# librosa/librosa

Measured on NVIDIA H100. Metric: mel-spectrogram frames/sec (n_fft=2048,hop=512,n_mels=128), higher is better.
Workload: dtype f32

## Files before the change

librosa_b200/csrc/api.cu:

```cuda
#include <cuda_runtime.h>
#include <math.h>
#include <stdlib.h>
#include <string.h>

#include <algorithm>

#include "aux_kernels.cuh"
#include "czt_kernel.cuh"
#include "feat_kernels.cuh"
#include "internal.h"
#include "mr_kernel.cuh"
#include "pitch_kernels.cuh"

using namespace b2l;

#define B2L_CASE(L) case L: return fwd_kernel_##L(variant, mode);
static FwdKernel fwd_kernel_for(int log2m, int variant, int mode) {
  switch (log2m) { B2L_FFT_SIZES(B2L_CASE) }
  return nullptr;
}
#undef B2L_CASE
#define B2L_CASE(L) case L: return inv_kernel_##L(variant);
static InvKernel inv_kernel_for(int log2m, int variant) {
  switch (log2m) { B2L_FFT_SIZES(B2L_CASE) }
  return nullptr;
}
#undef B2L_CASE
#define B2L_CASE(L) case L: return czt_kernel_##L();
static CztKernel czt_kernel_for(int log2p) {
  switch (log2p) { B2L_CZT_SIZES(B2L_CASE) }
  return nullptr;
}
#undef B2L_CASE
#define B2L_CASE(L) case L: return czt_inv_kernel_##L();
static CztInvKernel czt_inv_kernel_for(int log2p) {
  switch (log2p) { B2L_CZT_SIZES(B2L_CASE) }
  return nullptr;
}
#undef B2L_CASE

static int cta_variants(const HostFftCfg& cfg, int out[3]) {
  int n = 0;
  if (cfg.log2m >= 9 && cfg.log2m <= 11) out[n++] = 116;
  int nws[2];
  const int k = cfg.nw_options(nws);
  for (int i = 0; i < k; ++i) out[n++] = nws[i];
  return n;
}
static int variant_threads(int variant) { return variant == 116 ? 512 : variant * 32; }

enum Path { PATH_POW2, PATH_MR, PATH_CZT, PATH_NONE };
enum Entry {
  ENTRY_SPECTRUM,
  ENTRY_MEL,
  ENTRY_STATS,
};
static bool mr_enabled(const b2l_plan* p) {
  if (p->log2p == 0) return true;
  const char* e = getenv("B2L_MR");
  return !(e && *e) || atoi(e) != 0;
}
static Path route(const b2l_plan* p, Entry entry) {
  if (!p->czt) return PATH_POW2;
  switch (entry) {
    case ENTRY_SPECTRUM: return p->mr && mr_enabled(p) ? PATH_MR : PATH_CZT;
    case ENTRY_MEL: return p->mr ? PATH_MR : PATH_NONE;
    default: return PATH_NONE;
  }
}

static int frame_count(b2l_ctx* c, const b2l_plan* p, int64_t n_clips, int64_t n, int64_t y_stride, const float* d_y,
                       const void* d_out, long long* T) {
  if (p->ctx != c) return fail(B2L_ERR_INVALID, "plan belongs to another context");
  if (n_clips < 0 || n < 0 || y_stride < n) return fail(B2L_ERR_INVALID, "bad clip geometry");
  if (n > 0x7fffffffLL) return fail(B2L_ERR_UNSUPPORTED, "clips longer than 2^31-1 samples are not supported");
  *T = plan_frames(p, n);
  if (*T <= 0)
    return fail(B2L_ERR_INVALID, "n_fft=%d is too large for input signal of length=%lld", p->n_fft, (long long)n);
  if (n_clips == 0) *T = 0;
  else if (!d_y || !d_out) return fail(B2L_ERR_INVALID, "NULL device pointer");
  return B2L_OK;
}

struct StatsCall { StatsParams sp; const float* d_freq; };

static int run_forward(b2l_ctx* c, const b2l_plan* p, int mode, int log_mode, const float* d_y, int64_t n_clips,
                       int64_t n, int64_t y_stride, float2* out_c, float* out_r, const StatsCall* stats = nullptr) {
  long long T = 0;
  int rc = frame_count(c, p, n_clips, n, y_stride, d_y, mode == MODE_STFT ? (void*)out_c : (void*)out_r, &T);
  if (rc || T == 0) return rc;
  if (mode == MODE_MEL && p->n_mels == 0) return fail(B2L_ERR_INVALID, "plan has no mel stage");
  DeviceGuard g(c->device);

  HostFftCfg cfg(p->log2m);
  const int N = p->n_fft, M = N / 2;
  int variants[3];
  const int n_opt = cta_variants(cfg, variants);
  FwdArgs a;
  memset(&a, 0, sizeof(a));
  int variant = 0, ft = 0, halves = 1;
  size_t smem = 0;
  const b2l_plan::RowTable* rt = nullptr;
  for (int i = 0; i < n_opt && !variant; ++i) {
    const int v = variants[i];
    const int nh = v == 116 ? 2 : 1;
    const int nw = nh > 1 ? 16 : v;
    if (nw * 32 % (cfg.tpf * nh) != 0) continue;
    const int f = nw * 32 / nh / cfg.tpf;
    if (f < 1 || f > 32) continue;
    const long long span = (long long)(f - 1) * p->hop + N;
    if (span > 0x3fffffff) continue;
    const b2l_plan::RowTable* t = nullptr;
    if (mode == MODE_MEL) {
      rc = get_row_table(p, mel_rows_per_warp(f), &t);
      if (rc) return rc;
    }
    size_t off = 0;
    a.off_win = (int)off; off = align_up(off + (size_t)N * 4, 16);
    a.off_tw = (int)off; off = align_up(off + (size_t)cfg.tw_count(true) * 8, 16);
    a.off_bar = (int)off; off = align_up(off + 8 * nh, 16);
    if (t) {
      a.off_melw = (int)off; off = align_up(off + (size_t)t->w_count * 4, 16);
      a.off_melband = (int)off; off = align_up(off + (size_t)t->n_rows * sizeof(MelRow), 16);
    }
    if (mode == MODE_STATS) {
      a.off_melw = (int)off; off = align_up(off + (size_t)(M + 1) * 4, 16);
    }
    a.off_in = (int)(off = align_up(off, 128));
    a.in_stride = (int)align_up((size_t)span * 4, 128);
    off += (size_t)a.in_stride * nh;
    a.off_xbuf = (int)(off = align_up(off, 128));
    size_t xbytes = (size_t)f * cfg.xbuf_f2() * 8;
    if (mode == MODE_MEL || mode == MODE_STATS) {
      xbytes = (size_t)f * mel_group_stride(M, f) * 8 + (M < 128 ? (size_t)(M + 16) * 4 : 0);
    }
    a.xbuf_stride = (int)align_up(xbytes, 128);
    off += (size_t)a.xbuf_stride * nh;
    if (off > c->smem_optin) continue;
    variant = v;
    ft = f;
    halves = nh;
    smem = off;
    rt = t;
    a.in_floats = (int)span;
  }
  if (!variant)
    return fail(B2L_ERR_UNSUPPORTED, "hop_length=%d with n_fft=%d needs more shared memory than one SM has", p->hop,
                p->n_fft);

  a.y = d_y;
  a.clip_stride = y_stride;
  a.n = (int)n;
  a.n_clips = (int)n_clips;
  a.n_fft = N;
  a.hop = p->hop;
  a.pad = p->center ? N / 2 : 0;
  a.pad_mode = p->pad_mode;
  a.n_frames = (int)T;
  a.tiles_per_clip = (int)((T + ft - 1) / ft);
  a.total_tiles = (long long)a.tiles_per_clip * n_clips;
  a.tma_ok = (((uintptr_t)d_y & 15) == 0) && (y_stride % 4 == 0) && (a.in_floats % 4 == 0);
  a.window = p->d_win_fwd;
  a.tw = p->d_tw_fwd;
  a.twn = p->d_twn;
  a.out_c = out_c;
  a.out_r = out_r;
  a.power_mode = p->power_mode;
  a.power = p->power;
  a.n_mels = p->n_mels;
  if (mode == MODE_STATS) {
    if (!stats || !stats->d_freq) return fail(B2L_ERR_INVALID, "NULL frequency table");
    a.power_mode = 1;
    a.power = 1.0f;
    a.stats = stats->sp;
    a.mel_w = stats->d_freq;
    a.mel_w_count = M + 1;
  }
  if (rt) {
    a.mel_w_count = rt->w_count;
    a.mel_w = rt->d_w;
    a.mel_rows = rt->d_rows;
    a.n_mel_rows = rt->n_rows;
  }
  a.log_mode = log_mode ? 1 : 0;
  a.out_tiled = log_mode == 2 ? 1 : 0;
  a.amin = p->amin;
  a.db_sub = 10.0f * log10f(fmaxf(p->amin, fabsf(p->ref_value)));
  a.clip_max = c->d_clip_max;
  a.status = c->d_status;

  const FwdKernel fn = fwd_kernel_for(p->log2m, variant, mode);
  if (!fn) return fail(B2L_ERR_CUDA, "no forward kernel variant %d for n_fft=%d", variant, N);
  const int threads = variant_threads(variant);
  int occ = 0;
  if ((rc = blocks_per_sm(c, fn, threads, smem, &occ))) return rc;
  if (occ < 1) return fail(B2L_ERR_CUDA, "forward kernel does not fit on an SM (smem %zu)", smem);
  long long grid = (long long)c->sm_count * occ;
  const long long ctas_needed = (a.total_tiles + halves - 1) / halves;
  if (grid > ctas_needed) grid = ctas_needed;
  return launch(c, fn, (unsigned)grid, threads, smem, a);
}

static size_t czt_smem(const b2l_plan* p, const HostFftCfg& cfg, int G, bool forward) {
  const size_t bins = forward ? (size_t)(1 + p->n_fft / 2) : 0;
  return (size_t)((cfg.tw_count() + 15) & ~15) * 8 + (size_t)G * cfg.xbuf_f2() * 8 +
         ((size_t)(1 << p->log2p) + (size_t)((p->n_fft + 1) & ~1) + bins) * 8;
}

static int run_czt(b2l_ctx* c, const b2l_plan* p, int mode, const float* d_y, int64_t n_clips, int64_t n,
                   int64_t y_stride, float2* out_c, float* out_r) {
  long long T = 0;
  int rc = frame_count(c, p, n_clips, n, y_stride, d_y, mode == 0 ? (void*)out_c : (void*)out_r, &T);
  if (rc || T == 0) return rc;
  DeviceGuard g(c->device);
  HostFftCfg cfg(p->log2p);
  const int nw = cfg.czt_nw();
  const int G = nw * 32 / cfg.tpf;
  CztArgs a;
  memset(&a, 0, sizeof(a));
  a.y = d_y;
  a.clip_stride = y_stride;
  a.n = (int)n;
  a.n_clips = (int)n_clips;
  a.L = p->n_fft;
  a.hop = p->hop;
  a.pad = p->center ? p->n_fft / 2 : 0;
  a.pad_mode = p->pad_mode;
  a.n_frames = (int)T;
  a.n_bins = 1 + p->n_fft / 2;
  a.wb = p->d_czt_wb;
  a.bk = p->d_czt_bk;
  a.hf = p->d_czt_hf;
  a.out_c = out_c;
  a.out_r = out_r;
  a.mode = mode;
  a.power_mode = p->power_mode;
  a.power = p->power;
  a.status = c->d_status;
  const size_t smem = czt_smem(p, cfg, G, true);
  const CztKernel fn = czt_kernel_for(p->log2p);
  int occ = 0;
  if ((rc = blocks_per_sm(c, fn, nw * 32, c->smem_optin / 2 + 1, &occ))) return rc;
  if (smem > c->smem_optin) return fail(B2L_ERR_UNSUPPORTED, "n_fft=%d needs more shared memory than one SM has", p->n_fft);
  if (occ < 1) return fail(B2L_ERR_CUDA, "chirp-z kernel does not fit on an SM (smem %zu)", smem);
  const long long steps = ((long long)n_clips * ((T + 1) / 2) + G - 1) / G;
  long long grid = (long long)c->sm_count * occ;
  if (grid > steps) grid = steps;
  return launch(c, fn, (unsigned)grid, nw * 32, smem, a);
}

static int mr_block(const b2l_ctx* c, const b2l_plan* p, int n_mels, int mel_w_count, int fpw, int* nw, size_t* smem) {
  const size_t tables = mr_table_bytes(p->n_fft, p->mr_tw_count, n_mels, mel_w_count);
  const size_t per_warp = (size_t)2 * (p->n_fft / 2) * sizeof(float2) * (size_t)fpw;
  const size_t budget = (c->smem_optin + 1024) / 2 - 1024;
  int w = 16;
  while (w > 1 && tables + w * per_warp > budget) --w;
  if (tables + w * per_warp > c->smem_optin)
    return fail(B2L_ERR_UNSUPPORTED, "n_fft=%d needs more shared memory than one SM has", p->n_fft);
  *nw = w;
  *smem = tables + w * per_warp;
  return B2L_OK;
}

static int run_mr(b2l_ctx* c, const b2l_plan* p, int mode, int log_mode, const float* d_y, int64_t n_clips, int64_t n,
                  int64_t y_stride, float2* out_c, float* out_r) {
  long long T = 0;
  int rc = frame_count(c, p, n_clips, n, y_stride, d_y, mode == 0 ? (void*)out_c : (void*)out_r, &T);
  if (rc || T == 0) return rc;
  if (mode == 2 && p->n_mels == 0) return fail(B2L_ERR_INVALID, "plan has no mel stage");
  if (n_clips > 0x7fffffffLL || T > 0x7fffffffLL) return fail(B2L_ERR_UNSUPPORTED, "batch too large");
  DeviceGuard g(c->device);
  MrArgs a;
  memset(&a, 0, sizeof(a));
  a.y = d_y;
  a.clip_stride = y_stride;
  a.n = (int)n;
// ... 1032 lines not shown
```

librosa_b200/csrc/common.cuh:

```cuda
#pragma once
#include <cuda_runtime.h>
#include <stdint.h>

namespace b2l {

enum PadMode : int {
  PAD_CONSTANT = 0,
  PAD_EDGE = 1,
  PAD_REFLECT = 2,
  PAD_SYMMETRIC = 3,
  PAD_LINEAR_RAMP = 4,
  PAD_EMPTY = 5,
};

enum FwdMode : int {
  MODE_STFT = 0,
  MODE_MEL = 1,
  MODE_SPEC = 2,
  MODE_STATS = 3,
};

constexpr int kMrMaxPass = 12;

struct MelBand { int lo, len, off, pad; };
struct MelRow { unsigned short lo, quads; unsigned int off; };

template <int M, int FT>
struct MelLayout {
  static constexpr bool PAIR = (FT % 2) == 0 && FT >= 8;
  static constexpr int FP = PAIR ? FT / 2 : FT;
  static constexpr int H = 32 / FP;
  static constexpr int RSM = H < 4 ? 4 : H;
  static constexpr int XB = M + M / 32;
  static constexpr int GS = XB + ((((RSM - 2 * XB) % 32) + 32) % 32) / 2;
  static constexpr int RS = 2 * GS;
  static_assert(RS >= M + 4 && RS % 32 == RSM % 32 && RS % 4 == 0, "row stride");
};
__host__ __device__ inline int mel_rows_per_warp(int ft) { return 32 / (((ft % 2) == 0 && ft >= 8) ? ft / 2 : ft); }
__host__ __device__ inline int mel_group_stride(int m, int ft) {
  const int h = mel_rows_per_warp(ft), rsm = h < 4 ? 4 : h, xb = m + m / 32;
  return xb + ((((rsm - 2 * xb) % 32) + 32) % 32) / 2;
}

enum StatRow : int { STAT_CENTROID = 0, STAT_BANDWIDTH = 1, STAT_ROLLOFF = 2, STAT_FLATNESS = 3, STAT_RMS = 4, STAT_TOTAL = 5 };
constexpr int N_STATS = 6;
struct StatsParams {
  float roll_percent;
  float flat_amin, flat_power;
  float bw_p;
  int bw_norm;
  int frame_length;
  int want;
};

struct FwdArgs {
  const float* y;
  long long clip_stride;
  int n, n_clips;
  int n_fft, hop, pad, pad_mode, n_frames;
  int tiles_per_clip;
  long long total_tiles;
  int tma_ok;
  const float* window;
  const float2* tw;
  const float2* twn;
  float2* out_c;
  float* out_r;
  int power_mode;
  float power;
  int n_mels, mel_w_count;
  const float* mel_w;
  const MelRow* mel_rows;
  int n_mel_rows;
  int log_mode;
  int out_tiled;
  float amin, db_sub;
  unsigned int* clip_max;
  int* status;
  StatsParams stats;
  int off_win, off_tw, off_in, off_xbuf, off_melw, off_melband, off_bar;
  int in_stride, xbuf_stride;
  int in_floats;
};

struct InvArgs {
  const float2* D;
  long long d_clip_stride;
  int n_clips, n_frames;
  int n_fft, hop, start;
  int out_len;
  long long y_clip_stride;
  float* y;
  const float* window;
  const float* inv_wss;
  const float2* tw;
  const float2* twn;
  int frames_per_slot;
  int vec4;
  int off_win, off_tw, off_xbuf, off_acc;
  int xbuf_stride, acc_stride;
  int acc_floats;
};

__host__ __device__ inline unsigned int float_to_key(float f) {
#ifdef __CUDA_ARCH__
  unsigned int u = __float_as_uint(f);
#else
  union { float f; unsigned int u; } c; c.f = f; unsigned int u = c.u;
#endif
  return (u & 0x80000000u) ? ~u : (u | 0x80000000u);
}
__host__ __device__ inline float key_to_float(unsigned int k) {
  unsigned int u = (k & 0x80000000u) ? (k & 0x7fffffffu) : ~k;
#ifdef __CUDA_ARCH__
  return __uint_as_float(u);
#else
  union { float f; unsigned int u; } c; c.u = u; return c.f;
#endif
}

}
```

librosa_b200/csrc/fwd_inst.cu:

```cuda
#include "fwd_kernel.cuh"
#include "internal.h"

#ifndef B2L_LOG2M
#error "compile with -DB2L_LOG2M=<2..12>"
#endif

namespace b2l {
namespace {

template <int L, int TPF, int NW, int DUAL>
FwdKernel by_mode(int mode) {
  switch (mode) {
    case MODE_STFT: return fwd_kernel<L, TPF, NW, MODE_STFT, DUAL>;
    case MODE_MEL: return fwd_kernel<L, TPF, NW, MODE_MEL, DUAL>;
    case MODE_SPEC: return fwd_kernel<L, TPF, NW, MODE_SPEC, DUAL>;
    case MODE_STATS: return fwd_kernel<L, TPF, NW, MODE_STATS, DUAL>;
  }
  return nullptr;
}

template <int L>
FwdKernel variant_kernel(int variant, int mode) {
  constexpr int M = 1 << L;
  constexpr int TPF = M >= 32 ? M / 32 : 1;
  if constexpr (L >= 10) {
    if (variant == 16) return by_mode<L, TPF, 16, 1>(mode);
    if (variant == 8) return by_mode<L, TPF, 8, 1>(mode);
    if (variant == 116) return by_mode<L, TPF, 16, 2>(mode);
  } else {
    constexpr int NW = TPF > 16 ? 16 : TPF;
    if (variant == NW) return by_mode<L, TPF, NW, 1>(mode);
    if constexpr (L == 9) {
      if (variant == 116) return by_mode<L, TPF, 16, 2>(mode);
    }
  }
  return nullptr;
}

}

#define B2L_CAT2(a, b) a##b
#define B2L_CAT(a, b) B2L_CAT2(a, b)

FwdKernel B2L_CAT(fwd_kernel_, B2L_LOG2M)(int variant, int mode) { return variant_kernel<B2L_LOG2M>(variant, mode); }

}
```

librosa_b200/csrc/fwd_kernel.cuh:

```cuda
#pragma once
#include "common.cuh"
#include "fft_engine.cuh"
#include "stats.cuh"


namespace b2l {

__device__ __forceinline__ void mbar_init(uint64_t* bar, int count) {
  asm volatile("mbarrier.init.shared::cta.b64 [%0], %1;" ::"r"(smem_u32(bar)), "r"(count) : "memory");
}
__device__ __forceinline__ void fence_mbar_init() {
  asm volatile("fence.mbarrier_init.release.cluster;" ::: "memory");
}
__device__ __forceinline__ void fence_proxy_async() {
  asm volatile("fence.proxy.async.shared::cta;" ::: "memory");
}
__device__ __forceinline__ void mbar_expect_tx(uint64_t* bar, uint32_t bytes) {
  asm volatile("mbarrier.arrive.expect_tx.shared::cta.b64 _, [%0], %1;" ::"r"(smem_u32(bar)), "r"(bytes)
               : "memory");
}
__device__ __forceinline__ void mbar_wait(uint64_t* bar, uint32_t phase) {
  asm volatile(
      "{\n\t"
      ".reg .pred p;\n\t"
      "WAIT_%=:\n\t"
      "mbarrier.try_wait.parity.shared::cta.b64 p, [%0], %1;\n\t"
      "@p bra DONE_%=;\n\t"
      "bra WAIT_%=;\n\t"
      "DONE_%=:\n\t"
      "}" ::"r"(smem_u32(bar)), "r"(phase)
      : "memory");
}
__device__ __forceinline__ void tma_load_1d(void* dst_smem, const void* src_gmem, uint32_t bytes, uint64_t* bar) {
  asm volatile(
      "cp.async.bulk.shared::cluster.global.mbarrier::complete_tx::bytes [%0], [%1], %2, [%3];" ::"r"(
          smem_u32(dst_smem)),
      "l"(src_gmem), "r"(bytes), "r"(smem_u32(bar))
      : "memory");
}

__device__ __forceinline__ float load_padded(const float* __restrict__ y, int n, long long j, int mode, int pad) {
  if (j >= 0 && j < n) return __ldg(y + j);
  switch (mode) {
    case PAD_EDGE:
      return __ldg(y + (j < 0 ? 0 : n - 1));
    case PAD_REFLECT: {
      if (n == 1) return __ldg(y);
      long long P = 2LL * (n - 1);
      long long m = j % P;
      if (m < 0) m += P;
      if (m >= n) m = P - m;
      return __ldg(y + m);
    }
    case PAD_SYMMETRIC: {
      long long P = 2LL * n;
      long long m = j % P;
      if (m < 0) m += P;
      if (m >= n) m = P - 1 - m;
      return __ldg(y + m);
    }
    case PAD_LINEAR_RAMP: {
      long long d = j < 0 ? -j : j - (n - 1);
      float edge = __ldg(y + (j < 0 ? 0 : n - 1));
      long long i = pad - d;
      if (i <= 0) return 0.0f;
      return (float)((double)i * ((double)edge / (double)pad));
    }
    default:
      return 0.0f;
  }
}

static __device__ __noinline__ float power_from_sq(float p2, int power_mode, float power) {
  float mag = sqrtf(p2);
  return power_mode == 1 ? mag : powf(mag, power);
}
__device__ __forceinline__ float sqmag(float2 x) { return fmaf(x.x, x.x, x.y * x.y); }
__device__ __forceinline__ float db10(float x) { return 3.0102999566398120f * __log2f(x); }
__device__ __forceinline__ float sqrt_approx(float x) {
  float r;
  asm("sqrt.approx.f32 %0, %1;" : "=f"(r) : "f"(x));
  return r;
}

template <int M, int TPF, int C>
__device__ __forceinline__ int partner_slot(int t) {
  if constexpr (TPF % 32 == 0) {
    constexpr int WPG = TPF / 32;
    const int tl = t & 31, tw = t >> 5;
    const int row = tw + WPG * C;
    const int rows = M / 32;
    const int a = 33 * (rows - 1 - row) + 32 - tl;
    const int b = 33 * ((rows - row) & (rows - 1));
    return tl == 0 ? b : a;
  } else {
    const int k = t + TPF * C;
    return xphys((M - k) & (M - 1));
  }
}

template <int LOG2M, int TPF, int NW, int MODE, int NSPLIT>
__global__ void __launch_bounds__(NW * 32, 1) fwd_kernel(const FwdArgs a) {
  using Cfg = FftCfg<LOG2M, TPF>;
  constexpr int M = Cfg::M, N = 2 * M, PPT = Cfg::PPT;
  constexpr int NT = NW * 32;
  constexpr int NH = NSPLIT;
  constexpr bool DUAL = NSPLIT > 1;
  constexpr int HT = NT / NH;
  constexpr int HW = NW / NH;
  constexpr int FT = HT / TPF;
  static_assert(NW % NSPLIT == 0, "the warps are split evenly");
  static_assert(TPF <= 32 || NH + NT / TPF <= 15, "named barriers: 1..NH for the halves, then one per frame group");
  static_assert(FT >= 1 && FT <= 32, "tile must hold 1..32 frames");
  using ML = MelLayout<M, FT>;
  constexpr int H = ML::H;
  constexpr int NPAIR = PPT / 2;

  extern __shared__ __align__(128) unsigned char smem[];
  const int tid = threadIdx.x;
  const int half = DUAL ? tid / HT : 0;
  const int htid = tid - half * HT;
  float* s_win = reinterpret_cast<float*>(smem + a.off_win);
  float2* s_tw = reinterpret_cast<float2*>(smem + a.off_tw);
  float* s_melw = reinterpret_cast<float*>(smem + a.off_melw);
  MelRow* s_row = reinterpret_cast<MelRow*>(smem + a.off_melband);
  float* s_in = reinterpret_cast<float*>(smem + a.off_in + half * a.in_stride);
  float2* s_xall = reinterpret_cast<float2*>(smem + a.off_xbuf + half * a.xbuf_stride);
  float* s_p = reinterpret_cast<float*>(s_xall);
  uint64_t* s_bar = reinterpret_cast<uint64_t*>(smem + a.off_bar) + half;

  const int grp = htid / TPF;
  const int t = htid % TPF;
  const int gbar = 1 + NH + half * FT + grp;
  constexpr int GS = (MODE == MODE_MEL || MODE == MODE_STATS) ? ML::GS : Cfg::XBUF_F2;
  float2* xbuf = s_xall + grp * GS;
  float2* xb_t = xbuf + xphys(t);
  const float2* xb_neg = xbuf - xphys(t) + ((t & 31) == 0 ? 1 : 0);

  auto half_sync = [&]() {
    if constexpr (DUAL) asm volatile("bar.sync %0, %1;" ::"r"(half + 1), "n"(HT) : "memory");
    else __syncthreads();
  };

  for (int i = tid; i < N; i += NT) s_win[i] = a.window[i];
  for (int i = tid; i < Cfg::TW_COUNT_SPLIT; i += NT) s_tw[i] = a.tw[i];
  if constexpr (MODE == MODE_MEL) {
    for (int i = tid; i < a.mel_w_count; i += NT) s_melw[i] = a.mel_w[i];
    for (int i = tid; i < a.n_mel_rows; i += NT) s_row[i] = a.mel_rows[i];
  }
  if constexpr (MODE == MODE_STATS) {
    for (int i = tid; i < a.mel_w_count; i += NT) s_melw[i] = a.mel_w[i];
  }
  if (htid == 0) {
    mbar_init(s_bar, 1);
    fence_mbar_init();
  }
  __syncthreads();

  const int span = a.in_floats;
  const bool hop_even = (a.hop & 1) == 0;
  const float2 wt = __ldg(a.twn + t);
  auto unmix_tw = [&](auto C) -> float2 {
    constexpr int c = decltype(C)::value;
    if constexpr (c == 0) return wt;
    else return cmul(wt, make_float2(TwC<c, 2 * PPT>::re, TwC<c, 2 * PPT>::im));
  };

  enum { TILE_GATHER = 0, TILE_TMA = 1, TILE_TMA_ZERO = 2 };
  struct TileInfo { int clip, tix, kind, lead, valid; };
  auto describe = [&](int clip, int tix) -> TileInfo {
    TileInfo ti;
    ti.clip = clip;
    ti.tix = tix;
    const long long s0 = (long long)tix * FT * a.hop - a.pad;
    ti.lead = s0 < 0 ? (int)(-s0) : 0;
    const long long end = s0 + span;
    ti.valid = (int)((end > a.n ? (long long)a.n : end) - (s0 + ti.lead));
    if (!a.tma_ok || ((s0 + ti.lead) & 3) != 0) ti.kind = TILE_GATHER;
    else if (ti.lead == 0 && ti.valid == span) ti.kind = TILE_TMA;
    else if (a.pad_mode == PAD_CONSTANT && ti.valid > 0 && (ti.lead & 3) == 0 && (ti.valid & 3) == 0) ti.kind = TILE_TMA_ZERO;
    else ti.kind = TILE_GATHER;
    return ti;
  };
  auto prefetch = [&](const TileInfo& ti) {
    if (ti.clip < a.n_clips && ti.kind != TILE_GATHER && htid == 0) {
      const long long s0 = (long long)ti.tix * FT * a.hop - a.pad;
      fence_proxy_async();
      mbar_expect_tx(s_bar, (uint32_t)ti.valid * 4u);
      tma_load_1d(s_in + ti.lead, a.y + (long long)ti.clip * a.clip_stride + s0 + ti.lead, (uint32_t)ti.valid * 4u, s_bar);
    }
    if (ti.clip < a.n_clips && ti.kind == TILE_TMA_ZERO) {
      for (int i = htid; i < ti.lead; i += HT) s_in[i] = 0.0f;
      for (int i = ti.lead + ti.valid + htid; i < span; i += HT) s_in[i] = 0.0f;
    }
  };

  const int tile_step = (int)gridDim.x * NH;
  const int step_c = tile_step / a.tiles_per_clip, step_t = tile_step - step_c * a.tiles_per_clip;
  TileInfo cur;
  {
    const int first = (int)blockIdx.x * NH + half;
    cur = describe(first / a.tiles_per_clip, first % a.tiles_per_clip);
  }
  uint32_t phase = 0;
  prefetch(cur);

  constexpr bool ROWS = (MODE == MODE_MEL || MODE == MODE_STATS);
  float2 v[PPT];
  auto stage_and_fetch = [&](const TileInfo& ti) {
    if (ti.kind == TILE_GATHER) {
      const float* yc = a.y + (long long)ti.clip * a.clip_stride;
      const long long s0 = (long long)ti.tix * FT * a.hop - a.pad;
      for (int i = htid; i < span; i += HT) s_in[i] = load_padded(yc, a.n, s0 + i, a.pad_mode, a.pad);
      half_sync();
    } else {
      mbar_wait(s_bar, phase);
      phase ^= 1;
      if (ti.kind == TILE_TMA_ZERO) half_sync();
    }
    const float* fr = s_in + grp * a.hop;
    auto win = [&](auto S) {
      constexpr int off = pass0_offset<Cfg>(decltype(S)::value);
      return *reinterpret_cast<const float2*>(s_win + 2 * (t + off));
    };
    if (hop_even) {
      load_pass0_windowed<Cfg>(v, t, [&](int e) { return *reinterpret_cast<const float2*>(fr + 2 * e); }, win);
    } else {
      load_pass0_windowed<Cfg>(v, t, [&](int e) { return make_float2(fr[2 * e], fr[2 * e + 1]); }, win);
    }
  };
  auto advance = [&](const TileInfo& ti) -> TileInfo {
    int nc = ti.clip + step_c, nt = ti.tix + step_t;
    if (nt >= a.tiles_per_clip) { nt -= a.tiles_per_clip; ++nc; }
    return describe(nc, nt);
  };

  for (; cur.clip < a.n_clips;) {
    const int clip = cur.clip, t0 = cur.tix * FT;
    stage_and_fetch(cur);
    const TileInfo nxt = advance(cur);
    half_sync();
    prefetch(nxt);
    auto rows_consumed = [&]() {
      if constexpr (ROWS) half_sync();
    };

    fft_forward<Cfg, true, true>(v, t, gbar, xbuf, s_tw, rows_consumed);
    if constexpr (Cfg::NPASS == 1) rows_consumed();
    constexpr bool SHFL_UNMIX = TPF == 32 && (MODE == MODE_MEL || MODE == MODE_STATS);
    static_assert(!SHFL_UNMIX || (PPT == 32 && spectrum_offset<Cfg>(1) == 32), "v[q] = Z[t + 32q]");
    constexpr bool AFFINE_UNMIX = (TPF % 32 == 0) && (TPF > 32 || MODE == MODE_MEL || MODE == MODE_STATS);
    if constexpr (!SHFL_UNMIX) {
      if constexpr (Cfg::NPASS > 1) group_sync<TPF>(gbar);
      static_for<0, PPT>([&](auto S) {
        constexpr int slot = decltype(S)::value;
        constexpr int D = spectrum_offset<Cfg>(slot);
        if constexpr (D >= M / 2) {
          if constexpr (AFFINE_UNMIX && D % 32 == 0) sts_c64(smem_u32(xb_t) + 8u * (D + D / 32), v[slot]);
          else sts_c64(smem_u32(xbuf) + 8u * xphys(t + D), v[slot]);
        }
      });
      group_sync<TPF>(gbar);
    }
    auto pair_operands = [&](auto C, float2& A, float2& B) {
      constexpr int c = decltype(C)::value;
      constexpr int sa = slot_of_pair<Cfg>(c);
      static_assert(sa >= 0, "pair operand must be register resident");
      A = v[sa];
      if constexpr (SHFL_UNMIX) {
        const float2 send = t == 0 ? v[(32 - c) & 31] : v[31 - c];
        B.x = __shfl_sync(0xffffffffu, send.x, (32 - t) & 31);
        B.y = __shfl_sync(0xffffffffu, send.y, (32 - t) & 31);
      } else if constexpr (AFFINE_UNMIX) {
        constexpr int K = 33 * (M / 32 - 1 - (TPF / 32) * c) + 32;
        if constexpr (c == 0) B = t == 0 ? A : xb_neg[K];
        else B = xb_neg[K];
      } else {
        B = xbuf[partner_slot<M, TPF, c>(t)];
        if constexpr (c == 0) {
          if (t == 0) B = A;
        }
      }
    };
    auto middle_bin = [&]() -> float2 {
      if constexpr (SHFL_UNMIX) return v[PPT / 2];
      else return xbuf[xphys(M / 2)];
    };

    const int frame = t0 + grp;
    const bool frame_ok = frame < a.n_frames;
    if (frame_ok && !(fabsf(v[0].x) + fabsf(v[0].y) <= 3.0e38f)) *a.status = 1;

    if constexpr (MODE == MODE_STFT) {
      float2* orow = a.out_c + ((long long)clip * a.n_frames + frame) * (M + 1);
      static_for<0, NPAIR>([&](auto C) {
        const int k = t + TPF * decltype(C)::value;
        float2 A, B, xa, xb;
        pair_operands(C, A, B);
        r2c_pair(A, B, unmix_tw(C), xa, xb);
        stg_c64_if(orow + k, xa, frame_ok);
        stg_c64_if(orow + (M - k), xb, frame_ok);
      });
      if (t == 0) {
        float2 xa, xb;
        float2 zc = middle_bin();
        r2c_pair(zc, zc, make_float2(0.0f, -1.0f), xa, xb);
        stg_c64_if(orow + M / 2, xa, frame_ok);
      }
      group_sync<TPF>(gbar);
    } else {
      float pw[PPT + 1];
      static_for<0, NPAIR>([&](auto C) {
        constexpr int c = decltype(C)::value;
        float2 A, B, xa, xb;
        pair_operands(C, A, B);
        r2c_pair(A, B, unmix_tw(C), xa, xb);
        pw[2 * c] = sqmag(xa);
        pw[2 * c + 1] = sqmag(xb);
      });
      pw[PPT] = 0.0f;
      if (t == 0) {
        float2 xa, xb;
        float2 zc = middle_bin();
        r2c_pair(zc, zc, make_float2(0.0f, -1.0f), xa, xb);
        pw[PPT] = sqmag(xa);
      }
      if (MODE == MODE_STATS || a.power_mode == 1) {
        static_for<0, PPT + 1>([&](auto S) { pw[decltype(S)::value] = sqrt_approx(pw[decltype(S)::value]); });
      } else if (a.power_mode != 2) {
        static_for<0, PPT + 1>([&](auto S) {
          pw[decltype(S)::value] = power_from_sq(pw[decltype(S)::value], a.power_mode, a.power);
        });
      }
      if constexpr (MODE == MODE_SPEC) {
        float* orow = a.out_r + ((long long)clip * a.n_frames + frame) * (M + 1);
        if (frame_ok) {
          static_for<0, NPAIR>([&](auto C) {
            constexpr int c = decltype(C)::value;
            const int k = t + TPF * c;
            orow[k] = pw[2 * c];
            orow[M - k] = pw[2 * c + 1];
          });
          if (t == 0) orow[M / 2] = pw[PPT];
        }
        group_sync<TPF>(gbar);
      } else {
        constexpr int RS = ML::RS;
        group_sync<TPF>(gbar);
        float* prow = reinterpret_cast<float*>(xbuf);
        static_for<0, NPAIR>([&](auto C) {
          constexpr int c = decltype(C)::value;
          const int k = t + TPF * c;
          prow[k] = pw[2 * c];
          prow[M - k] = pw[2 * c + 1];
        });
        if (t == 0) {
          prow[M / 2] = pw[PPT];
          prow[M + 1] = 0.0f;
          prow[M + 2] = 0.0f;
          prow[M + 3] = 0.0f;
        }
        half_sync();
        if constexpr (MODE == MODE_STATS) {
          const int hwarp = htid >> 5, lane = htid & 31;
          for (int f = hwarp; f < FT; f += HW) {
            bool negative;
            const float r = frame_stats(s_p + f * RS, s_melw, M + 1, lane, a.stats, &negative);
            if (lane < N_STATS && t0 + f < a.n_frames)
              a.out_r[((long long)clip * N_STATS + lane) * a.n_frames + t0 + f] = r;
          }
        } else {
          constexpr int FP = ML::FP;
          constexpr bool PAIR = ML::PAIR;
          const int hwarp = htid >> 5, lane = htid & 31;
          const int fp = lane & (FP - 1), j = lane / FP;
          const bool ok_a = (t0 + fp) < a.n_frames;
          const bool ok_b = PAIR && (t0 + fp + FP) < a.n_frames;
          float wmax = -INFINITY;
          const float* pbase = s_p + fp * RS;
          const long long orow = a.out_tiled ? 64 : a.n_frames;
          float* obase = a.out_tiled
                             ? a.out_r + ((long long)clip * ((a.n_frames + 63) >> 6) + (t0 >> 6)) * a.n_mels * 64 + (t0 & 63) + fp
                             : a.out_r + (long long)clip * a.n_mels * a.n_frames + t0 + fp;
          const int n_items = a.n_mel_rows / H;
          MelRow row_nx = s_row[(hwarp < n_items ? hwarp * H : 0) + j];
          for (int item = hwarp; item < n_items; item += HW) {
            const int m = item * H + j;
            const MelRow row = row_nx;
            const int item_nx = item + HW;
            row_nx = s_row[(item_nx < n_items ? item_nx * H : 0) + j];
            const float4* wp = reinterpret_cast<const float4*>(s_melw + row.off);
            const float4* pa = reinterpret_cast<const float4*>(pbase + row.lo);
            const float4* wend = wp + row.quads;
            float a0 = 0.0f, a1 = 0.0f, b0 = 0.0f, b1 = 0.0f;
            if constexpr (PAIR) {
              const float4* pb = pa + (FP * RS) / 4;
#pragma unroll 2
              for (; wp != wend; ++wp, ++pa, ++pb) {
                const float4 w = *wp, x = *pa, y = *pb;
                a0 = fmaf(w.x, x.x, a0);
                b0 = fmaf(w.x, y.x, b0);
                a1 = fmaf(w.y, x.y, a1);
                b1 = fmaf(w.y, y.y, b1);
                a0 = fmaf(w.z, x.z, a0);
                b0 = fmaf(w.z, y.z, b0);
                a1 = fmaf(w.w, x.w, a1);
                b1 = fmaf(w.w, y.w, b1);
              }
            } else {
#pragma unroll 2
              for (; wp != wend; ++wp, ++pa) {
                const float4 w = *wp, x = *pa;
                a0 = fmaf(w.x, x.x, a0);
                a1 = fmaf(w.y, x.y, a1);
                a0 = fmaf(w.z, x.z, a0);
                a1 = fmaf(w.w, x.w, a1);
              }
            }
            float va = a0 + a1, vb = b0 + b1;
            if (m < a.n_mels) {
              if (a.log_mode) {
                va = db10(fmaxf(a.amin, va)) - a.db_sub;
                if (ok_a) wmax = fmaxf(wmax, va);
                if constexpr (PAIR) {
                  vb = db10(fmaxf(a.amin, vb)) - a.db_sub;
                  if (ok_b) wmax = fmaxf(wmax, vb);
                }
              }
              float* o = obase + (long long)m * orow;
              if (ok_a) o[0] = va;
              if (ok_b) o[FP] = vb;
            }
          }
          if (a.log_mode) {
#pragma unroll
            for (int o = 16; o > 0; o >>= 1) wmax = fmaxf(wmax, __shfl_xor_sync(0xffffffffu, wmax, o));
            if (lane == 0 && wmax > -INFINITY) atomicMax(a.clip_max + clip, float_to_key(wmax));
          }
        }
      }
    }
    cur = nxt;
  }
}

}
```

librosa_b200/csrc/internal.h:

```cpp
#pragma once
#include <cuda_runtime.h>
#include <stdint.h>

#include <map>
#include <set>
#include <tuple>
#include <vector>

#include "../../include/b2l.h"
#include "common.cuh"
#include "fft_engine.cuh"

namespace b2l {

#define B2L_FFT_SIZES(X) X(2) X(3) X(4) X(5) X(6) X(7) X(8) X(9) X(10) X(11) X(12)
#define B2L_CZT_SIZES(X) X(5) X(6) X(7) X(8) X(9) X(10) X(11) X(12)
constexpr int kMinLog2M = 2, kMaxLog2M = 12;

struct CztArgs;
struct CztInvArgs;
typedef void (*FwdKernel)(FwdArgs);
typedef void (*InvKernel)(InvArgs);
typedef void (*CztKernel)(CztArgs);
typedef void (*CztInvKernel)(CztInvArgs);

#define B2L_DECL_FFT(L) FwdKernel fwd_kernel_##L(int variant, int mode); InvKernel inv_kernel_##L(int variant);
#define B2L_DECL_CZT(L) CztKernel czt_kernel_##L(); CztInvKernel czt_inv_kernel_##L();
B2L_FFT_SIZES(B2L_DECL_FFT)
B2L_CZT_SIZES(B2L_DECL_CZT)
#undef B2L_DECL_FFT
#undef B2L_DECL_CZT

struct HostFftCfg {
  int log2m, M, tpf, ppt, logp, npass;
  explicit HostFftCfg(int l2m) {
    log2m = l2m;
    M = 1 << l2m;
    tpf = M >= 32 ? M / 32 : 1;
    ppt = M / tpf;
    logp = 0;
    while ((1 << logp) < ppt) ++logp;
    npass = ppt == 1 ? 1 : (log2m + logp - 1) / logp;
  }
  int log_radix(int s) const { int left = log2m - s * logp; return left >= logp ? logp : left; }
  int radix(int s) const { return 1 << log_radix(s); }
  int sublen(int s) const { return 1 << (s * logp); }
  bool split_pass(int s, bool split) const { return split && tw_split_pass(log2m, s, radix(s)); }
  int tw_rows(int s, bool split) const { return split_pass(s, split) ? kTwSplitRows : radix(s) - 1; }
  int tw_offset(int s, bool split = false) const {
    int off = 0;
    for (int q = 1; q < s; ++q) off += tw_rows(q, split) * sublen(q);
    return off;
  }
  int tw_count(bool split = false) const { return tw_offset(npass, split); }
  int xbuf_f2() const { return M + M / 32; }
  int czt_nw() const { return log2m >= 10 ? 16 : (tpf > 16 ? 16 : tpf); }
  int nw_options(int out[2]) const {
    if (log2m >= 10) { out[0] = 16; out[1] = 8; return 2; }
    out[0] = tpf >= 1 ? (tpf > 16 ? 16 : tpf) : 1;
    return 1;
  }
};

int fail(int code, const char* fmt, ...);

#define CUDA_TRY(expr)                                                                        \
  do {                                                                                        \
    cudaError_t _e = (expr);                                                                  \
    if (_e != cudaSuccess) {                                                                  \
      cudaGetLastError();                                                                     \
      return fail(_e == cudaErrorMemoryAllocation ? B2L_ERR_OOM : B2L_ERR_CUDA, "%s: %s (%s:%d)", #expr, \
                  cudaGetErrorString(_e), __FILE__, __LINE__);                                \
    }                                                                                         \
  } while (0)

}

struct b2l_ctx {
  int device = 0;
  int sm_count = 0;
  size_t smem_optin = 0;
  cudaStream_t stream = nullptr;
  uint64_t launches = 0;
  struct ncclComm* comm = nullptr;
  int rank = 0, world = 1;
  unsigned int* d_clip_max = nullptr;
  int* d_status = nullptr;
  float* d_scratch = nullptr;
  size_t scratch_bytes = 0;
  size_t clip_max_cap = 0;
  std::set<const void*> smem_limit_set;
  std::map<std::tuple<const void*, int, size_t>, int> occupancy;
  std::vector<void*> stage_bufs;
  std::vector<cudaEvent_t> stage_evs;
};

struct b2l_plan {
  b2l_ctx* ctx = nullptr;
  int n_fft = 0, hop = 0, center = 0, pad_mode = 0, log2m = 0;
  mutable std::vector<void*> allocs;
  float* d_win_fwd = nullptr;
  float* d_win_inv = nullptr;
  float2* d_tw = nullptr;
  float2* d_tw_fwd = nullptr;
  float2* d_twn = nullptr;
  int tw_count = 0;
  int n_mels = 0, mel_w_count = 0;
  float* d_mel_w = nullptr;
  b2l::MelBand* d_band = nullptr;
  float* d_mel_wT = nullptr;
  std::vector<b2l::MelBand> h_band;
  std::vector<float> h_mel_w;
// ... 84 lines not shown
```

Before: 317.5 million.

## Add warp-specialized mel kernel with mbarrier rings for n_fft=2048

```diff
diff --git a/librosa_b200/csrc/api.cu b/librosa_b200/csrc/api.cu
--- a/librosa_b200/csrc/api.cu
+++ b/librosa_b200/csrc/api.cu
@@ -101,7 +101,37 @@
   int variant = 0, ft = 0, halves = 1;
   size_t smem = 0;
   const b2l_plan::RowTable* rt = nullptr;
-  for (int i = 0; i < n_opt && !variant; ++i) {
+  FwdKernel fn = mode == MODE_MEL && p->log2m == 10 ? fwd_mel_ws_kernel_10() : nullptr;
+  bool ws = false;
+  if (fn) {
+    const int f = MelWs::FT;
+    const long long span = (long long)(f - 1) * p->hop + N;
+    const b2l_plan::RowTable* t = nullptr;
+    if ((rc = get_row_table(p, mel_rows_per_warp(f), &t))) return rc;
+    size_t off = 0;
+    a.off_win = (int)off; off = align_up(off + (size_t)N * 4, 16);
+    a.off_tw = (int)off; off = align_up(off + (size_t)cfg.tw_count(true) * 8, 16);
+    a.off_bar = (int)off; off = align_up(off + 8 * MelWs::NBAR, 16);
+    a.off_melw = (int)off; off = align_up(off + (size_t)t->w_count * 4, 16);
+    a.off_melband = (int)off; off = align_up(off + (size_t)t->n_rows * sizeof(MelRow), 16);
+    a.off_in = (int)(off = align_up(off, 128));
+    a.in_stride = (int)align_up((size_t)span * 4, 128);
+    off += (size_t)a.in_stride * MelWs::NS;
+    a.off_xbuf = (int)(off = align_up(off, 128));
+    off += (size_t)MelWs::NF * cfg.xbuf_f2() * 8;
+    a.off_rows = (int)(off = align_up(off, 128));
+    off += (size_t)MelWs::NR * MelWs::FT * mel_ws_row_stride(M) * 4;
+    if (span <= 0x3fffffff && off <= c->smem_optin) {
+      ws = true;
+      ft = f;
+      smem = off;
+      rt = t;
+      a.in_floats = (int)span;
+    } else {
+      fn = nullptr;
+    }
+  }
+  for (int i = 0; i < n_opt && !ws && !variant; ++i) {
     const int v = variants[i];
     const int nh = v == 116 ? 2 : 1;
     const int nw = nh > 1 ? 16 : v;
@@ -144,7 +174,7 @@
     rt = t;
     a.in_floats = (int)span;
   }
-  if (!variant)
+  if (!ws && !variant)
     return fail(B2L_ERR_UNSUPPORTED, "hop_length=%d with n_fft=%d needs more shared memory than one SM has", p->hop,
                 p->n_fft);
 
@@ -189,9 +219,9 @@
   a.clip_max = c->d_clip_max;
   a.status = c->d_status;
 
-  const FwdKernel fn = fwd_kernel_for(p->log2m, variant, mode);
+  if (!fn) fn = fwd_kernel_for(p->log2m, variant, mode);
   if (!fn) return fail(B2L_ERR_CUDA, "no forward kernel variant %d for n_fft=%d", variant, N);
-  const int threads = variant_threads(variant);
+  const int threads = ws ? MelWs::NW * 32 : variant_threads(variant);
   int occ = 0;
   if ((rc = blocks_per_sm(c, fn, threads, smem, &occ))) return rc;
   if (occ < 1) return fail(B2L_ERR_CUDA, "forward kernel does not fit on an SM (smem %zu)", smem);
diff --git a/librosa_b200/csrc/common.cuh b/librosa_b200/csrc/common.cuh
--- a/librosa_b200/csrc/common.cuh
+++ b/librosa_b200/csrc/common.cuh
@@ -42,6 +42,19 @@
   return xb + ((((rsm - 2 * xb) % 32) + 32) % 32) / 2;
 }
 
+struct MelWs {
+  static constexpr int NF = 11;
+  static constexpr int NMEL = 5;
+  static constexpr int NW = NF + NMEL;
+  static constexpr int FT = 8;
+  static constexpr int NS = 2;
+  static constexpr int NR = 2;
+  static constexpr int NBAR = 2 * NS + 2 * NR;
+};
+__host__ __device__ constexpr int mel_ws_row_stride(int m) {
+  return (m + 4) + ((((8 - (m + 4)) % 32) + 32) % 32);
+}
+
 enum StatRow : int { STAT_CENTROID = 0, STAT_BANDWIDTH = 1, STAT_ROLLOFF = 2, STAT_FLATNESS = 3, STAT_RMS = 4, STAT_TOTAL = 5 };
 constexpr int N_STATS = 6;
 struct StatsParams {
@@ -79,6 +92,7 @@
   int* status;
   StatsParams stats;
   int off_win, off_tw, off_in, off_xbuf, off_melw, off_melband, off_bar;
+  int off_rows;
   int in_stride, xbuf_stride;
   int in_floats;
 };
diff --git a/librosa_b200/csrc/fwd_inst.cu b/librosa_b200/csrc/fwd_inst.cu
--- a/librosa_b200/csrc/fwd_inst.cu
+++ b/librosa_b200/csrc/fwd_inst.cu
@@ -1,5 +1,10 @@
 #include "fwd_kernel.cuh"
+#include "fwd_mel_ws.cuh"
 #include "internal.h"
+
+#ifndef B2L_MEL_WS
+#define B2L_MEL_WS 1
+#endif
 
 #ifndef B2L_LOG2M
 #error "compile with -DB2L_LOG2M=<2..12>"
@@ -44,4 +49,8 @@
 
 FwdKernel B2L_CAT(fwd_kernel_, B2L_LOG2M)(int variant, int mode) { return variant_kernel<B2L_LOG2M>(variant, mode); }
 
+#if B2L_LOG2M == 10
+FwdKernel fwd_mel_ws_kernel_10() { return B2L_MEL_WS ? fwd_mel_ws_kernel<10> : nullptr; }
+#endif
+
 }
diff --git a/librosa_b200/csrc/fwd_kernel.cuh b/librosa_b200/csrc/fwd_kernel.cuh
--- a/librosa_b200/csrc/fwd_kernel.cuh
+++ b/librosa_b200/csrc/fwd_kernel.cuh
@@ -98,6 +98,101 @@
     return xphys((M - k) & (M - 1));
   }
 }
+
+enum { TILE_GATHER = 0, TILE_TMA = 1, TILE_TMA_ZERO = 2 };
+struct TileInfo { int clip, tix, kind, lead, valid; };
+__device__ __forceinline__ TileInfo describe_tile(const FwdArgs& a, int ft, int span, int clip, int tix) {
+  TileInfo ti;
+  ti.clip = clip;
+  ti.tix = tix;
+  const long long s0 = (long long)tix * ft * a.hop - a.pad;
+  ti.lead = s0 < 0 ? (int)(-s0) : 0;
+  const long long end = s0 + span;
+  ti.valid = (int)((end > a.n ? (long long)a.n : end) - (s0 + ti.lead));
+  if (!a.tma_ok || ((s0 + ti.lead) & 3) != 0) ti.kind = TILE_GATHER;
+  else if (ti.lead == 0 && ti.valid == span) ti.kind = TILE_TMA;
+  else if (a.pad_mode == PAD_CONSTANT && ti.valid > 0 && (ti.lead & 3) == 0 && (ti.valid & 3) == 0) ti.kind = TILE_TMA_ZERO;
+  else ti.kind = TILE_GATHER;
+  return ti;
+}
+
+template <int M, int FT, int RS>
+__device__ __forceinline__ void mel_project_tile(const FwdArgs& a, const float* s_p, const float* s_melw,
+                                                 const MelRow* s_row, int clip, int t0, int w, int nw, int lane) {
+  using ML = MelLayout<M, FT>;
+  constexpr int H = ML::H;
+  constexpr int FP = ML::FP;
+  constexpr bool PAIR = ML::PAIR;
+  static_assert(RS >= M + 4 && RS % 32 == ML::RSM % 32 && RS % 4 == 0, "row stride");
+  const int fp = lane & (FP - 1), j = lane / FP;
+  const bool ok_a = (t0 + fp) < a.n_frames;
+  const bool ok_b = PAIR && (t0 + fp + FP) < a.n_frames;
+  float wmax = -INFINITY;
+  const float* pbase = s_p + fp * RS;
+  const long long orow = a.out_tiled ? 64 : a.n_frames;
+  float* obase = a.out_tiled
+                     ? a.out_r + ((long long)clip * ((a.n_frames + 63) >> 6) + (t0 >> 6)) * a.n_mels * 64 + (t0 & 63) + fp
+                     : a.out_r + (long long)clip * a.n_mels * a.n_frames + t0 + fp;
+  const int n_items = a.n_mel_rows / H;
+  MelRow row_nx = s_row[(w < n_items ? w * H : 0) + j];
+  for (int item = w; item < n_items; item += nw) {
+    const int m = item * H + j;
+    const MelRow row = row_nx;
+    const int item_nx = item + nw;
+    row_nx = s_row[(item_nx < n_items ? item_nx * H : 0) + j];
+    const float4* wp = reinterpret_cast<const float4*>(s_melw + row.off);
+    const float4* pa = reinterpret_cast<const float4*>(pbase + row.lo);
+    const float4* wend = wp + row.quads;
+    float a0 = 0.0f, a1 = 0.0f, b0 = 0.0f, b1 = 0.0f;
+    if constexpr (PAIR) {
+      const float4* pb = pa + (FP * RS) / 4;
+#pragma unroll 2
+      for (; wp != wend; ++wp, ++pa, ++pb) {
+        const float4 w = *wp, x = *pa, y = *pb;
+        a0 = fmaf(w.x, x.x, a0);
+        b0 = fmaf(w.x, y.x, b0);
+        a1 = fmaf(w.y, x.y, a1);
+        b1 = fmaf(w.y, y.y, b1);
+        a0 = fmaf(w.z, x.z, a0);
+        b0 = fmaf(w.z, y.z, b0);
+        a1 = fmaf(w.w, x.w, a1);
+        b1 = fmaf(w.w, y.w, b1);
+      }
+    } else {
+#pragma unroll 2
+      for (; wp != wend; ++wp, ++pa) {
+        const float4 w = *wp, x = *pa;
+        a0 = fmaf(w.x, x.x, a0);
+        a1 = fmaf(w.y, x.y, a1);
+        a0 = fmaf(w.z, x.z, a0);
+        a1 = fmaf(w.w, x.w, a1);
+      }
+    }
+    float va = a0 + a1, vb = b0 + b1;
+    if (m < a.n_mels) {
+      if (a.log_mode) {
+        va = db10(fmaxf(a.amin, va)) - a.db_sub;
+        if (ok_a) wmax = fmaxf(wmax, va);
+        if constexpr (PAIR) {
+          vb = db10(fmaxf(a.amin, vb)) - a.db_sub;
+          if (ok_b) wmax = fmaxf(wmax, vb);
+        }
+      }
+      float* o = obase + (long long)m * orow;
+      if (ok_a) o[0] = va;
+      if (ok_b) o[FP] = vb;
+    }
+  }
+  if (a.log_mode) {
+#pragma unroll
+    for (int o = 16; o > 0; o >>= 1) wmax = fmaxf(wmax, __shfl_xor_sync(0xffffffffu, wmax, o));
+    if (lane == 0 && wmax > -INFINITY) atomicMax(a.clip_max + clip, float_to_key(wmax));
+  }
+}
+
+#ifndef B2L_MEL_ABLATE
+#define B2L_MEL_ABLATE 0
+#endif
 
 template <int LOG2M, int TPF, int NW, int MODE, int NSPLIT>
 __global__ void __launch_bounds__(NW * 32, 1) fwd_kernel(const FwdArgs a) {
@@ -113,7 +208,6 @@
   static_assert(TPF <= 32 || NH + NT / TPF <= 15, "named barriers: 1..NH for the halves, then one per frame group");
   static_assert(FT >= 1 && FT <= 32, "tile must hold 1..32 frames");
   using ML = MelLayout<M, FT>;
-  constexpr int H = ML::H;
   constexpr int NPAIR = PPT / 2;
 
   extern __shared__ __align__(128) unsigned char smem[];
@@ -166,22 +260,7 @@
     else return cmul(wt, make_float2(TwC<c, 2 * PPT>::re, TwC<c, 2 * PPT>::im));
   };
 
-  enum { TILE_GATHER = 0, TILE_TMA = 1, TILE_TMA_ZERO = 2 };
-  struct TileInfo { int clip, tix, kind, lead, valid; };
-  auto describe = [&](int clip, int tix) -> TileInfo {
-    TileInfo ti;
-    ti.clip = clip;
-    ti.tix = tix;
-    const long long s0 = (long long)tix * FT * a.hop - a.pad;
-    ti.lead = s0 < 0 ? (int)(-s0) : 0;
-    const long long end = s0 + span;
-    ti.valid = (int)((end > a.n ? (long long)a.n : end) - (s0 + ti.lead));
-    if (!a.tma_ok || ((s0 + ti.lead) & 3) != 0) ti.kind = TILE_GATHER;
-    else if (ti.lead == 0 && ti.valid == span) ti.kind = TILE_TMA;
-    else if (a.pad_mode == PAD_CONSTANT && ti.valid > 0 && (ti.lead & 3) == 0 && (ti.valid & 3) == 0) ti.kind = TILE_TMA_ZERO;
-    else ti.kind = TILE_GATHER;
-    return ti;
-  };
+  auto describe = [&](int clip, int tix) -> TileInfo { return describe_tile(a, FT, span, clip, tix); };
   auto prefetch = [&](const TileInfo& ti) {
     if (ti.clip < a.n_clips && ti.kind != TILE_GATHER && htid == 0) {
       const long long s0 = (long long)ti.tix * FT * a.hop - a.pad;
@@ -205,7 +284,8 @@
   uint32_t phase = 0;
   prefetch(cur);
 
-  constexpr bool ROWS = (MODE == MODE_MEL || MODE == MODE_STATS);
+  constexpr int ABLATE = MODE == MODE_MEL ? B2L_MEL_ABLATE : 0;
+  constexpr bool ROWS = (MODE == MODE_MEL && ABLATE != 1) || MODE == MODE_STATS;
   float2 v[PPT];
   auto stage_and_fetch = [&](const TileInfo& ti) {
     if (ti.kind == TILE_GATHER) {
@@ -344,6 +424,12 @@
           if (t == 0) orow[M / 2] = pw[PPT];
         }
         group_sync<TPF>(gbar);
+      } else if constexpr (ABLATE == 1) {
+        if (frame < 0) {
+          float* orow = a.out_r + (long long)clip * a.n_frames * (M + 1);
+          static_for<0, PPT + 1>([&](auto S) { orow[t + TPF * decltype(S)::value] = pw[decltype(S)::value]; });
+        }
+        group_sync<TPF>(gbar);
       } else {
         constexpr int RS = ML::RS;
         group_sync<TPF>(gbar);
@@ -369,74 +455,8 @@
             if (lane < N_STATS && t0 + f < a.n_frames)
               a.out_r[((long long)clip * N_STATS + lane) * a.n_frames + t0 + f] = r;
           }
-        } else {
-          constexpr int FP = ML::FP;
-          constexpr bool PAIR = ML::PAIR;
-          const int hwarp = htid >> 5, lane = htid & 31;
-          const int fp = lane & (FP - 1), j = lane / FP;
-          const bool ok_a = (t0 + fp) < a.n_frames;
-          const bool ok_b = PAIR && (t0 + fp + FP) < a.n_frames;
-          float wmax = -INFINITY;
-          const float* pbase = s_p + fp * RS;
-          const long long orow = a.out_tiled ? 64 : a.n_frames;
-          float* obase = a.out_tiled
-                             ? a.out_r + ((long long)clip * ((a.n_frames + 63) >> 6) + (t0 >> 6)) * a.n_mels * 64 + (t0 & 63) + fp
-                             : a.out_r + (long long)clip * a.n_mels * a.n_frames + t0 + fp;
-          const int n_items = a.n_mel_rows / H;
-          MelRow row_nx = s_row[(hwarp < n_items ? hwarp * H : 0) + j];
-          for (int item = hwarp; item < n_items; item += HW) {
-            const int m = item * H + j;
-            const MelRow row = row_nx;
-            const int item_nx = item + HW;
-            row_nx = s_row[(item_nx < n_items ? item_nx * H : 0) + j];
-            const float4* wp = reinterpret_cast<const float4*>(s_melw + row.off);
-            const float4* pa = reinterpret_cast<const float4*>(pbase + row.lo);
-            const float4* wend = wp + row.quads;
-            float a0 = 0.0f, a1 = 0.0f, b0 = 0.0f, b1 = 0.0f;
-            if constexpr (PAIR) {
-              const float4* pb = pa + (FP * RS) / 4;
-#pragma unroll 2
-              for (; wp != wend; ++wp, ++pa, ++pb) {
-                const float4 w = *wp, x = *pa, y = *pb;
-                a0 = fmaf(w.x, x.x, a0);
-                b0 = fmaf(w.x, y.x, b0);
-                a1 = fmaf(w.y, x.y, a1);
-                b1 = fmaf(w.y, y.y, b1);
-                a0 = fmaf(w.z, x.z, a0);
-                b0 = fmaf(w.z, y.z, b0);
-                a1 = fmaf(w.w, x.w, a1);
-                b1 = fmaf(w.w, y.w, b1);
-              }
-            } else {
-#pragma unroll 2
-              for (; wp != wend; ++wp, ++pa) {
-                const float4 w = *wp, x = *pa;
-                a0 = fmaf(w.x, x.x, a0);
-                a1 = fmaf(w.y, x.y, a1);
-                a0 = fmaf(w.z, x.z, a0);
-                a1 = fmaf(w.w, x.w, a1);
-              }
-            }
-            float va = a0 + a1, vb = b0 + b1;
-            if (m < a.n_mels) {
-              if (a.log_mode) {
-                va = db10(fmaxf(a.amin, va)) - a.db_sub;
-                if (ok_a) wmax = fmaxf(wmax, va);
-                if constexpr (PAIR) {
-                  vb = db10(fmaxf(a.amin, vb)) - a.db_sub;
-                  if (ok_b) wmax = fmaxf(wmax, vb);
-                }
-              }
-              float* o = obase + (long long)m * orow;
-              if (ok_a) o[0] = va;
-              if (ok_b) o[FP] = vb;
-            }
-          }
-          if (a.log_mode) {
-#pragma unroll
-            for (int o = 16; o > 0; o >>= 1) wmax = fmaxf(wmax, __shfl_xor_sync(0xffffffffu, wmax, o));
-            if (lane == 0 && wmax > -INFINITY) atomicMax(a.clip_max + clip, float_to_key(wmax));
-          }
+        } else if constexpr (ABLATE != 2) {
+          mel_project_tile<M, FT, RS>(a, s_p, s_melw, s_row, clip, t0, htid >> 5, HW, htid & 31);
         }
       }
     }
diff --git a/librosa_b200/csrc/fwd_mel_ws.cuh b/librosa_b200/csrc/fwd_mel_ws.cuh
--- /dev/null
+++ b/librosa_b200/csrc/fwd_mel_ws.cuh
@@ -0,0 +1,195 @@
+#pragma once
+#include "fwd_kernel.cuh"
+
+namespace b2l {
+
+__device__ __forceinline__ void mbar_arrive(uint64_t* bar) {
+  asm volatile("mbarrier.arrive.shared::cta.b64 _, [%0];" ::"r"(smem_u32(bar)) : "memory");
+}
+
+template <int LOG2M>
+__global__ void __launch_bounds__(MelWs::NW * 32, 1) fwd_mel_ws_kernel(const FwdArgs a) {
+  using Cfg = FftCfg<LOG2M, 32>;
+  constexpr int M = Cfg::M, N = 2 * M, PPT = Cfg::PPT, TPF = 32;
+  constexpr int NF = MelWs::NF, NMEL = MelWs::NMEL, NT = MelWs::NW * 32;
+  constexpr int FT = MelWs::FT, NS = MelWs::NS, NR = MelWs::NR;
+  constexpr int RS = mel_ws_row_stride(M);
+  constexpr int NPAIR = PPT / 2;
+  static_assert(PPT == 32 && Cfg::NPASS == 2 && spectrum_offset<Cfg>(1) == 32, "v[q] = Z[t + 32q] after two passes");
+  static_assert(RS % 32 == MelLayout<M, FT>::RSM % 32, "row stride follows MelLayout's bank rule");
+  static_assert((NS & (NS - 1)) == 0 && (NR & (NR - 1)) == 0, "ring depths are powers of two");
+
+  extern __shared__ __align__(128) unsigned char smem[];
+  const int tid = threadIdx.x, warp = tid >> 5, lane = tid & 31;
+  float* s_win = reinterpret_cast<float*>(smem + a.off_win);
+  float2* s_tw = reinterpret_cast<float2*>(smem + a.off_tw);
+  float* s_melw = reinterpret_cast<float*>(smem + a.off_melw);
+  MelRow* s_row = reinterpret_cast<MelRow*>(smem + a.off_melband);
+  float* s_rows = reinterpret_cast<float*>(smem + a.off_rows);
+  uint64_t* full = reinterpret_cast<uint64_t*>(smem + a.off_bar);
+  uint64_t* empty = full + NS;
+  uint64_t* rfull = empty + NS;
+  uint64_t* rempty = rfull + NR;
+  auto s_in = [&](int slot) { return reinterpret_cast<float*>(smem + a.off_in + slot * a.in_stride); };
+
+  for (int i = tid; i < N; i += NT) s_win[i] = a.window[i];
+  for (int i = tid; i < Cfg::TW_COUNT_SPLIT; i += NT) s_tw[i] = a.tw[i];
+  for (int i = tid; i < a.mel_w_count; i += NT) s_melw[i] = a.mel_w[i];
+  for (int i = tid; i < a.n_mel_rows; i += NT) s_row[i] = a.mel_rows[i];
+  for (int i = tid; i < NR * FT * 3; i += NT) s_rows[(i / 3) * RS + M + 1 + i % 3] = 0.0f;
+  if (tid == 0) {
+    for (int s = 0; s < NS; ++s) {
+      mbar_init(full + s, 1);
+      mbar_init(empty + s, FT);
+    }
+    for (int r = 0; r < NR; ++r) {
+      mbar_init(rfull + r, FT);
+      mbar_init(rempty + r, NMEL);
+    }
+    fence_mbar_init();
+  }
+  __syncthreads();
+
+  const int step_c = (int)gridDim.x / a.tiles_per_clip, step_t = (int)gridDim.x - step_c * a.tiles_per_clip;
+  auto advance = [&](const TileInfo& ti) -> TileInfo {
+    int nc = ti.clip + step_c, nt = ti.tix + step_t;
+    if (nt >= a.tiles_per_clip) { nt -= a.tiles_per_clip; ++nc; }
+    return describe_tile(a, FT, a.in_floats, nc, nt);
+  };
+  const TileInfo first =
+      describe_tile(a, FT, a.in_floats, (int)blockIdx.x / a.tiles_per_clip, (int)blockIdx.x % a.tiles_per_clip);
+
+  if (warp < NF) {
+    const int t = lane;
+    float2* xbuf = reinterpret_cast<float2*>(smem + a.off_xbuf) + warp * Cfg::XBUF_F2;
+    const bool hop_even = (a.hop & 1) == 0;
+    const float2 wt = __ldg(a.twn + t);
+    auto unmix_tw = [&](auto C) -> float2 {
+      constexpr int c = decltype(C)::value;
+      if constexpr (c == 0) return wt;
+      else return cmul(wt, make_float2(TwC<c, 2 * PPT>::re, TwC<c, 2 * PPT>::im));
+    };
+    int i = warp / FT, j = warp % FT;
+    TileInfo ti = first;
+    for (int k = 0; k < i; ++k) ti = advance(ti);
+    float2 v[PPT];
+    while (ti.clip < a.n_clips) {
+      const int slot = i & (NS - 1);
+      mbar_wait(full + slot, (uint32_t)(i / NS) & 1u);
+      const float* fr = s_in(slot) + j * a.hop;
+      auto win = [&](auto S) {
+        constexpr int off = pass0_offset<Cfg>(decltype(S)::value);
+        return *reinterpret_cast<const float2*>(s_win + 2 * (t + off));
+      };
+      if (hop_even) {
+        load_pass0_windowed<Cfg>(v, t, [&](int e) { return *reinterpret_cast<const float2*>(fr + 2 * e); }, win);
+      } else {
+        load_pass0_windowed<Cfg>(v, t, [&](int e) { return make_float2(fr[2 * e], fr[2 * e + 1]); }, win);
+      }
+      __syncwarp();
+      if (lane == 0) mbar_arrive(empty + slot);
+
+      fft_forward<Cfg, true, true>(v, t, 0, xbuf, s_tw);
+
+      const int frame = ti.tix * FT + j;
+      if (frame < a.n_frames && !(fabsf(v[0].x) + fabsf(v[0].y) <= 3.0e38f)) *a.status = 1;
+
+      float pw[PPT + 1];
+      static_for<0, NPAIR>([&](auto C) {
+        constexpr int c = decltype(C)::value;
+        constexpr int sa = slot_of_pair<Cfg>(c);
+        float2 B, xa, xb;
+        const float2 A = v[sa];
+        const float2 send = t == 0 ? v[(32 - c) & 31] : v[31 - c];
+        B.x = __shfl_sync(0xffffffffu, send.x, (32 - t) & 31);
+        B.y = __shfl_sync(0xffffffffu, send.y, (32 - t) & 31);
+        r2c_pair(A, B, unmix_tw(C), xa, xb);
+        pw[2 * c] = sqmag(xa);
+        pw[2 * c + 1] = sqmag(xb);
+      });
+      pw[PPT] = 0.0f;
+      if (t == 0) {
+        float2 xa, xb;
+        const float2 zc = v[PPT / 2];
+        r2c_pair(zc, zc, make_float2(0.0f, -1.0f), xa, xb);
+        pw[PPT] = sqmag(xa);
+      }
+      if (a.power_mode == 1) {
+        static_for<0, PPT + 1>([&](auto S) { pw[decltype(S)::value] = sqrt_approx(pw[decltype(S)::value]); });
+      } else if (a.power_mode != 2) {
+        static_for<0, PPT + 1>([&](auto S) {
+          pw[decltype(S)::value] = power_from_sq(pw[decltype(S)::value], a.power_mode, a.power);
+        });
+      }
+
+      const int r = i & (NR - 1);
+      mbar_wait(rempty + r, ((uint32_t)(i / NR) & 1u) ^ 1u);
+      float* prow = s_rows + (r * FT + j) * RS;
+      static_for<0, NPAIR>([&](auto C) {
+        constexpr int c = decltype(C)::value;
+        const int k = t + TPF * c;
+        prow[k] = pw[2 * c];
+        prow[M - k] = pw[2 * c + 1];
+      });
+      if (t == 0) prow[M / 2] = pw[PPT];
+      __syncwarp();
+      if (lane == 0) mbar_arrive(rfull + r);
+
+      j += NF % FT;
+      int di = NF / FT;
+      if (j >= FT) { j -= FT; ++di; }
+      i += di;
+      for (; di > 0; --di) ti = advance(ti);
+    }
+  } else {
+    const int mw = warp - NF;
+    const int span = a.in_floats;
+    auto produce = [&](const TileInfo& ti, int slot) {
+      float* dst = s_in(slot);
+      const long long s0 = (long long)ti.tix * FT * a.hop - a.pad;
+      if (ti.kind == TILE_GATHER) {
+        const float* yc = a.y + (long long)ti.clip * a.clip_stride;
+        for (int e = lane; e < span; e += 32) dst[e] = load_padded(yc, a.n, s0 + e, a.pad_mode, a.pad);
+        __syncwarp();
+        if (lane == 0) mbar_arrive(full + slot);
+      } else {
+        if (ti.kind == TILE_TMA_ZERO) {
+          for (int e = lane; e < ti.lead; e += 32) dst[e] = 0.0f;
+          for (int e = ti.lead + ti.valid + lane; e < span; e += 32) dst[e] = 0.0f;
+        }
+        __syncwarp();
+        if (lane == 0) {
+          fence_proxy_async();
+          mbar_expect_tx(full + slot, (uint32_t)ti.valid * 4u);
+          tma_load_1d(dst + ti.lead, a.y + (long long)ti.clip * a.clip_stride + s0 + ti.lead, (uint32_t)ti.valid * 4u,
+                      full + slot);
+        }
+      }
+    };
+    TileInfo nxt = first;
+    if (mw == 0) {
+      for (int s = 0; s < NS && nxt.clip < a.n_clips; ++s) {
+        produce(nxt, s);
+        nxt = advance(nxt);
+      }
+    }
+    TileInfo ti = first;
+    for (int i = 0; ti.clip < a.n_clips; ++i) {
+      if (mw == 0 && nxt.clip < a.n_clips) {
+        const int slot = i & (NS - 1);
+        mbar_wait(empty + slot, (uint32_t)(i / NS) & 1u);
+        produce(nxt, slot);
+        nxt = advance(nxt);
+      }
+      const int r = i & (NR - 1);
+      mbar_wait(rfull + r, (uint32_t)(i / NR) & 1u);
+      mel_project_tile<M, FT, RS>(a, s_rows + r * FT * RS, s_melw, s_row, ti.clip, ti.tix * FT, NMEL - 1 - mw, NMEL,
+                                  lane);
+      __syncwarp();
+      if (lane == 0) mbar_arrive(rempty + r);
+      ti = advance(ti);
+    }
+  }
+}
+
+}
diff --git a/librosa_b200/csrc/internal.h b/librosa_b200/csrc/internal.h
--- a/librosa_b200/csrc/internal.h
+++ b/librosa_b200/csrc/internal.h
@@ -28,6 +28,7 @@
 #define B2L_DECL_CZT(L) CztKernel czt_kernel_##L(); CztInvKernel czt_inv_kernel_##L();
 B2L_FFT_SIZES(B2L_DECL_FFT)
 B2L_CZT_SIZES(B2L_DECL_CZT)
+FwdKernel fwd_mel_ws_kernel_10();
 #undef B2L_DECL_FFT
 #undef B2L_DECL_CZT
 
```

Result: faster. 321.7 million (median of 6 runs) (+1.3%).
